# Zhiyu014/GNN-UDS

Hardware: AMD Instinct MI355X
Metric: graph-steps/sec (forward rollout), |V|=10k |E|=12k d=64 (higher is better)
Workload: dtype f32 storage/accumulate, GEMM operands as bf16 hi+lo split (3 MFMA products)

## Files before the change

### gnn_uds_amd/csrc/kernels_fused_ws.hpp

```cpp
#pragma once
#include "kernels_fused.hpp"

namespace uds {

#ifndef UDS_WS_NY
#define UDS_WS_NY 4
#endif
#ifndef UDS_WS_SLOTS
#define UDS_WS_SLOTS 4
#endif
constexpr int WS_NY = UDS_WS_NY, WS_NX = FUSED_WAVES - WS_NY;
#ifdef UDS_WS_YG
constexpr int WS_YG = UDS_WS_NY;
#else
constexpr int WS_YG = 0;
#endif
constexpr int WS_SLOTS = UDS_WS_SLOTS;
#ifndef UDS_WS_PRE
#define UDS_WS_PRE 0
#endif
constexpr int WS_PRE = UDS_WS_PRE;
static_assert(WS_PRE % WS_SLOTS == 0, "WS_PRE must be a multiple of WS_SLOTS");
#ifndef UDS_WS_XPRIO
#define UDS_WS_XPRIO 1
#endif
static_assert(WS_NY >= 2 && WS_NY <= 4, "2 .. 4 waves multiply the primary rows");

inline int64_t fused_ws_lds_bytes(int p_cap, int q_cap, int meta_cap) {
  return 4 * ((int64_t)meta_cap + 4 * p_cap + 3 * FUSED_D + FUSED_H + 2 * (int64_t)q_cap * SEC_STRIDE + 2 * (int64_t)p_cap * FUSED_D);
}

template <int IMM>
__device__ __forceinline__ void ws_gld16(f32x4 &dst, const float *base, unsigned voff) {
  asm volatile("global_load_dwordx4 %0, %1, %2 offset:%3" : "=v"(dst) : "v"(voff), "s"(base), "n"(IMM) : "memory");
}
__device__ __forceinline__ void ws_pin4(f32x4 &a0, f32x4 &a1, f32x4 &a2, f32x4 &a3) {
  asm volatile("" : "+v"(a0), "+v"(a1), "+v"(a2), "+v"(a3));
}
__device__ __forceinline__ void row8_max4(const float (&in)[4], float (&out)[4]) {
  asm("s_nop 1\n\t" UDS_DPP4_FIRST("v_max_f32_dpp", "quad_perm:[1,0,3,2]") UDS_DPP4("v_max_f32_dpp", "quad_perm:[2,3,0,1]")
      UDS_DPP4("v_max_f32_dpp", "row_half_mirror")
      : "=&v"(out[0]), "=&v"(out[1]), "=&v"(out[2]), "=&v"(out[3])
      : "v"(in[0]), "v"(in[1]), "v"(in[2]), "v"(in[3]));
}
__device__ __forceinline__ void row8_sum4(const float (&in)[4], float (&out)[4]) {
  asm("s_nop 1\n\t" UDS_DPP4_FIRST("v_add_f32_dpp", "quad_perm:[1,0,3,2]") UDS_DPP4("v_add_f32_dpp", "quad_perm:[2,3,0,1]")
      UDS_DPP4("v_add_f32_dpp", "row_half_mirror")
      : "=&v"(out[0]), "=&v"(out[1]), "=&v"(out[2]), "=&v"(out[3])
      : "v"(in[0]), "v"(in[1]), "v"(in[2]), "v"(in[3]));
}
template <int HI>
__device__ __forceinline__ unsigned ws_add_half(unsigned pk, unsigned base) {
  unsigned r;
  if (HI) asm("v_add_u32_sdwa %0, %1, %2 dst_sel:DWORD dst_unused:UNUSED_PAD src0_sel:WORD_1 src1_sel:DWORD" : "=v"(r) : "v"(pk), "v"(base));
  else asm("v_add_u32_sdwa %0, %1, %2 dst_sel:DWORD dst_unused:UNUSED_PAD src0_sel:WORD_0 src1_sel:DWORD" : "=v"(r) : "v"(pk), "v"(base));
  return r;
}
__device__ __forceinline__ void ws_vmcnt(int n) {
  switch (n) {
    case 0: asm volatile("s_waitcnt vmcnt(0)" ::: "memory"); break;
    case 1: asm volatile("s_waitcnt vmcnt(1)" ::: "memory"); break;
    case 2: asm volatile("s_waitcnt vmcnt(2)" ::: "memory"); break;
    case 3: asm volatile("s_waitcnt vmcnt(3)" ::: "memory"); break;
    case 4: asm volatile("s_waitcnt vmcnt(4)" ::: "memory"); break;
    case 5: asm volatile("s_waitcnt vmcnt(5)" ::: "memory"); break;
    case 6: asm volatile("s_waitcnt vmcnt(6)" ::: "memory"); break;
    case 7: asm volatile("s_waitcnt vmcnt(7)" ::: "memory"); break;
    default: asm volatile("s_waitcnt vmcnt(8)" ::: "memory"); break;
  }
}

template <int ACT>
__global__ __launch_bounds__(FUSED_WAVES * 64, 2) void k_fused_ws(FusedArgs a) {
  constexpr int NT = FUSED_WAVES * 64, NY = WS_NY, NX = WS_NX;
  constexpr int FP = 64, FS = 64;
  constexpr int KT_S = FS / 32, MB_S = FUSED_H / 16;
  constexpr int KT_X = FP / 32, KT_B = KT_X + 1, MB_B = FUSED_D / 16;
  constexpr int U = FUSED_U;
  constexpr int PJ = (8 + NY - 1) / NY;
  constexpr int SJ = (16 + NX - 1) / NX;
  extern __shared__ __attribute__((aligned(16))) int32_t smem[];

  const int tid = threadIdx.x, lane = tid & 63;
  const int wave = __builtin_amdgcn_readfirstlane(tid >> 6);
#ifdef UDS_WS_PAIR_SAME
  static_assert(NY == 4, "UDS_WS_PAIR_SAME assumes 4 + 4");
  const bool team_y = (wave & 3) < 2;
  const int yw = (wave & 1) + 2 * (wave >> 2), xw = ((wave & 3) - 2) + 2 * (wave >> 2);
#else
  const bool team_y = wave < NY;
  const int yw = wave, xw = wave - NY;
#endif
  const int r16 = lane & 15, qd = lane >> 4;
  const int c16 = r16, rs = qd;

  const int W = gridDim.x, b = blockIdx.x;
  const int q8 = W / 8, r8 = W % 8, xcd = b % 8;
  const int w = (xcd < r8 ? xcd * (q8 + 1) : r8 * (q8 + 1) + (xcd - r8) * q8) + b / 8;
  const int tile = w % a.n_tiles;
  const int chunk_id = w / a.n_tiles;
  const int s_begin = chunk_id * a.chunk;
  const int s_end = min(a.S, (chunk_id + 1) * a.chunk);
  const int sd = __builtin_amdgcn_readfirstlane(a.hdr[tile * TILE_HDR_INTS + 6]);
  if (!((a.side_mask >> sd) & 1)) return;
  const FusedSide &S_ = a.side[sd];

  float *s_self = reinterpret_cast<float *>(smem + a.meta_cap);
  float *s_nbr = s_self + 2 * a.p_cap;
  float *attn = s_nbr + 2 * a.p_cap;
  float *sec = attn + 3 * FUSED_D + FUSED_H;
  float *hx = sec + 2 * a.q_cap * SEC_STRIDE;
  const int sec_buf = a.q_cap * SEC_STRIDE, hx_buf = a.p_cap * FUSED_D;

  {
    const uint4 *src = reinterpret_cast<const uint4 *>(a.blocks + (int64_t)tile * a.meta_cap);
    uint4 *dst = reinterpret_cast<uint4 *>(smem);
    for (int i = tid; i < a.meta_cap / 4; i += NT) dst[i] = src[i];
  }
  if (tid < FUSED_D) {
    attn[tid] = S_.a_self[tid] * 1.44269504088896340736f;
    attn[FUSED_D + tid] = S_.a_nbr[tid] * 1.44269504088896340736f;
    if (tid < FUSED_H) attn[2 * FUSED_D + tid] = S_.b_small ? S_.b_small[tid] : 0.f;
    attn[2 * FUSED_D + FUSED_H + tid] = S_.b_out ? S_.b_out[tid] : 0.f;
  }
  __syncthreads();
  const int n_own = __builtin_amdgcn_readfirstlane(smem[0]), n_prim = __builtin_amdgcn_readfirstlane(smem[1]),
            n_sec = __builtin_amdgcn_readfirstlane(smem[2]), flags = __builtin_amdgcn_readfirstlane(smem[3]),
            n_ovf = __builtin_amdgcn_readfirstlane(smem[4]), n_adj = __builtin_amdgcn_readfirstlane(smem[5]),
            inc_width = __builtin_amdgcn_readfirstlane(smem[7]);
  const EllOffsets off = ell_offsets(n_own, n_prim, n_sec, flags, n_ovf, n_adj);
  const int32_t *prim_ids = smem + off.prim;
  const int32_t *sec_ids = smem + off.sec;
  const uint32_t *inc_loc = reinterpret_cast<const uint32_t *>(smem + off.inc_loc);
  int32_t *inc_w = smem + off.inc_w;
  const f32x4 *inc_val4 = reinterpret_cast<const f32x4 *>(inc_w);
  const unsigned char *adj_b = reinterpret_cast<const unsigned char *>(smem + off.adj);
  const int32_t *ovf_ptr = smem + off.ovf_ptr, *ovf_loc = smem + off.ovf_loc;
  int32_t *ovf_w = smem + off.ovf_w;
  const int32_t *adj_ptr = smem + off.adj_ptr, *adj_loc = smem + off.adj_loc;

  for (int i = tid; i < ELL_INC * n_prim; i += NT) {
    const int k = inc_w[i];
    reinterpret_cast<float *>(inc_w)[i] = k >= 0 ? S_.ne_val[k] : 0.f;
  }
  if (flags & ELL_FLAG_INC_OVF)
    for (int i = tid; i < n_ovf; i += NT) reinterpret_cast<float *>(ovf_w)[i] = S_.ne_val[ovf_w[i]];
  const float *ovf_val = reinterpret_cast<const float *>(ovf_w);

#ifdef UDS_PHASE_TIMING
  unsigned long long tm_[8] = {0, 0, 0, 0, 0, 0, 0, 0}, tl_ = clock64();
  const unsigned long long rt0_ = __builtin_amdgcn_s_memrealtime(), mt0_ = tl_;
#define WS_STAMP(k) do { const unsigned long long n_ = clock64(); tm_[k] += n_ - tl_; tl_ = n_; } while (0)
#define WS_DUMP() do { if (a.dbg && lane == 0) { unsigned long long *o = a.dbg + ((size_t)blockIdx.x * 8 + wave) * 16; \
    for (int q_ = 0; q_ < 7; ++q_) o[q_] = tm_[q_]; o[12] = wave; \
    o[15] = ((__builtin_amdgcn_s_memrealtime() - rt0_) << 32) | ((clock64() - mt0_) & 0xffffffffull); \
    o[7] = 1ull | ((unsigned long long)sd << 8) | ((unsigned long long)n_own << 16) | ((unsigned long long)n_prim << 32) | ((unsigned long long)n_sec << 48); } } while (0)
#else
#define WS_STAMP(k) do { } while (0)
#define WS_DUMP() do { } while (0)
#endif
  const int64_t sec_stride = (int64_t)S_.n_sec_glob * FS, prim_stride = (int64_t)S_.n_prim_glob * FP;
  const int n_snap = s_end - s_begin;

  __syncthreads();
  if (team_y) {
#ifndef UDS_WS_MFMA16
    typedef float f32x16 __attribute__((ext_vector_type(16)));
    constexpr int KT32 = (FP + FUSED_H) / 16, KX32 = FP / 16, MB32 = FUSED_D / 32;
    static_assert(NY == 4, "one 32-row block per Y wave: four waves cover p_cap = 128");
    const int n32 = lane & 31, hf = lane >> 5;
    bf16x8 wh[KT32][MB32], wl[KT32][MB32];
#pragma unroll
    for (int t = 0; t < KT32; ++t)
#pragma unroll
      for (int m = 0; m < MB32; ++m) {
        wh[t][m] = __builtin_bit_cast(bf16x8, S_.w_big32[((t * MB32 + m) * 2 + 0) * 64 + lane]);
        wl[t][m] = __builtin_bit_cast(bf16x8, S_.w_big32[((t * MB32 + m) * 2 + 1) * 64 + lane]);
      }
    const int lrow = 32 * yw + n32;
    const bool valid = lrow < n_prim;
    const int lr = min(lrow, n_prim - 1);
    const unsigned prow = (unsigned)prim_ids[lr] * FP + 8u * hf;
    f32x4 pp[2 * KX32];
    const bool has_rem = S_.rem != nullptr;
    const unsigned rrow = (unsigned)prim_ids[lr] * FUSED_H + 8u * hf;
    f32x4 rm[4] = {f32x4{0.f, 0.f, 0.f, 0.f}, f32x4{0.f, 0.f, 0.f, 0.f}, f32x4{0.f, 0.f, 0.f, 0.f}, f32x4{0.f, 0.f, 0.f, 0.f}};
    const int64_t rem_stride = (int64_t)S_.n_prim_glob * FUSED_H;
    const unsigned ag_locs = inc_loc[lr];
    const f32x4 ag_vals = inc_val4[lr];
    __builtin_amdgcn_s_waitcnt(0x0F70);
    if (n_snap > 0) {
      const float *base = S_.prim_in + s_begin * prim_stride;
      static_for<2 * KX32>([&](auto i_) {
        constexpr int i = decltype(i_)::value;
        pp[i] = *reinterpret_cast<const f32x4 *>(base + prow + 16 * (i >> 1) + 4 * (i & 1));
      });
      if (has_rem) {
        const float *rb = S_.rem + s_begin * rem_stride + rrow;
        rm[0] = *reinterpret_cast<const f32x4 *>(rb);
        rm[1] = *reinterpret_cast<const f32x4 *>(rb + 4);
        rm[2] = *reinterpret_cast<const f32x4 *>(rb + 16);
        rm[3] = *reinterpret_cast<const f32x4 *>(rb + 20);
      }
    }
    WS_STAMP(0);
    lds_barrier();

    auto mfma3_32 = [&](const bf16x8 &a_h, const bf16x8 &a_l, const bf16x8 &d_h, const bf16x8 &d_l, f32x16 acc) __attribute__((always_inline)) {
      acc = __builtin_amdgcn_mfma_f32_32x32x16_bf16(a_h, d_l, acc, 0, 0, 0);
      acc = __builtin_amdgcn_mfma_f32_32x32x16_bf16(a_l, d_h, acc, 0, 0, 0);
      acc = __builtin_amdgcn_mfma_f32_32x32x16_bf16(a_h, d_h, acc, 0, 0, 0);
      return acc;
    };
    for (int k = 0; k <= n_snap; ++k) {
#ifdef UDS_WS_ABL_NO_P2
      if (false) {
#else
      if (k < n_snap && 32 * yw < n_prim) {
#endif
        const bool more = k + 1 < n_snap;
        const float *next = S_.prim_in + (s_begin + k + 1) * prim_stride;
        const float *secr = sec + (k & 1) * sec_buf;
        float *hxw = hx + (k & 1) * hx_buf;
        float *ssw = s_self + (k & 1) * a.p_cap, *snw = s_nbr + (k & 1) * a.p_cap;
        bf16x8 dh[KT32], dl[KT32];
        static_for<KX32>([&](auto t_) {
          constexpr int t = decltype(t_)::value;
          const f32x4 u0 = pp[2 * t], u1 = pp[2 * t + 1];
          split8(make_float4(u0[0], u0[1], u0[2], u0[3]), make_float4(u1[0], u1[1], u1[2], u1[3]), dh[t], dl[t]);
        });
        if (more)
          static_for<2 * KX32>([&](auto i_) {
            constexpr int i = decltype(i_)::value;
            pp[i] = *reinterpret_cast<const f32x4 *>(next + prow + 16 * (i >> 1) + 4 * (i & 1));
          });
        f32x16 acc[MB32];
#pragma unroll
        for (int m = 0; m < MB32; ++m)
#pragma unroll
          for (int r = 0; r < 16; ++r) acc[m][r] = 0.f;
#pragma unroll
        for (int t = 0; t < KX32; ++t)
#pragma unroll
          for (int m = 0; m < MB32; ++m) acc[m] = mfma3_32(wh[t][m], wl[t][m], dh[t], dl[t], acc[m]);
        float4 g0 = make_float4(rm[0][0], rm[0][1], rm[0][2], rm[0][3]), g1 = make_float4(rm[1][0], rm[1][1], rm[1][2], rm[1][3]),
               g2 = make_float4(rm[2][0], rm[2][1], rm[2][2], rm[2][3]), g3 = make_float4(rm[3][0], rm[3][1], rm[3][2], rm[3][3]);
        if (more && has_rem) {
          const float *rb = S_.rem + (s_begin + k + 1) * rem_stride + rrow;
          rm[0] = *reinterpret_cast<const f32x4 *>(rb);
          rm[1] = *reinterpret_cast<const f32x4 *>(rb + 4);
          rm[2] = *reinterpret_cast<const f32x4 *>(rb + 16);
          rm[3] = *reinterpret_cast<const f32x4 *>(rb + 20);
        }
        auto fma4 = [&](float4 &g, float wv, const float4 &u) { g.x = fmaf(wv, u.x, g.x); g.y = fmaf(wv, u.y, g.y); g.z = fmaf(wv, u.z, g.z); g.w = fmaf(wv, u.w, g.w); };
        auto add_row = [&](unsigned la, float wa) {
          const float *ra = secr + la * SEC_STRIDE + 8 * hf;
          const float4 u0 = *reinterpret_cast<const float4 *>(ra), u1 = *reinterpret_cast<const float4 *>(ra + 4);
          const float4 u2 = *reinterpret_cast<const float4 *>(ra + 16), u3 = *reinterpret_cast<const float4 *>(ra + 20);
          fma4(g0, wa, u0); fma4(g1, wa, u1); fma4(g2, wa, u2); fma4(g3, wa, u3);
        };
        add_row(ag_locs & 0xffu, ag_vals[0]);
        add_row((ag_locs >> 8) & 0xffu, ag_vals[1]);
        if (inc_width > 2) {
          add_row((ag_locs >> 16) & 0xffu, ag_vals[2]);
          add_row(ag_locs >> 24, ag_vals[3]);
        }
        if (flags & ELL_FLAG_INC_OVF)
          for (int p = ovf_ptr[lr]; p < ovf_ptr[lr + 1]; ++p) add_row((unsigned)ovf_loc[p], ovf_val[p]);
        split8(g0, g1, dh[KX32], dl[KX32]);
        split8(g2, g3, dh[KX32 + 1], dl[KX32 + 1]);
#pragma unroll
        for (int t = KX32; t < KT32; ++t)
#pragma unroll
          for (int m = 0; m < MB32; ++m) acc[m] = mfma3_32(wh[t][m], wl[t][m], dh[t], dl[t], acc[m]);
        float ps = 0.f, pn = 0.f;
#pragma unroll
        for (int m = 0; m < MB32; ++m)
#pragma unroll
          for (int gq = 0; gq < 4; ++gq) {
            const f32x4 as4 = *reinterpret_cast<const f32x4 *>(attn + 32 * m + 8 * gq + 4 * hf);
            const f32x4 an4 = *reinterpret_cast<const f32x4 *>(attn + FUSED_D + 32 * m + 8 * gq + 4 * hf);
#pragma unroll
            for (int q = 0; q < 4; ++q) {
              ps = fmaf(acc[m][4 * gq + q], as4[q], ps);
              pn = fmaf(acc[m][4 * gq + q], an4[q], pn);
            }
          }
        ps += __shfl_xor(ps, 32);
        pn += __shfl_xor(pn, 32);
        if (valid) {
          if (hf == 0) {
            ssw[lrow] = ps;
            snw[lrow] = pn;
          }
#pragma unroll
          for (int m = 0; m < MB32; ++m)
#pragma unroll
            for (int gq = 0; gq < 4; ++gq) {
              const f32x4 o = {acc[m][4 * gq], acc[m][4 * gq + 1], acc[m][4 * gq + 2], acc[m][4 * gq + 3]};
              *reinterpret_cast<f32x4 *>(hxw + lrow * FUSED_D + (((8 * m + 2 * gq + hf) ^ (lrow & 7)) << 2)) = o;
            }
        }
      }
      WS_STAMP(1);
      lds_barrier();
      WS_STAMP(2);
    }
    WS_DUMP();
#else
    bf16x8 wbh[KT_B][MB_B], wbl[KT_B][MB_B];
#pragma unroll
    for (int t = 0; t < KT_B; ++t)
#pragma unroll
      for (int m = 0; m < MB_B; ++m) {
        wbh[t][m] = __builtin_bit_cast(bf16x8, S_.w_big[((t * MB_B + m) * 2 + 0) * 64 + lane]);
        wbl[t][m] = __builtin_bit_cast(bf16x8, S_.w_big[((t * MB_B + m) * 2 + 1) * 64 + lane]);
      }
    unsigned prow[PJ];
#pragma unroll
    for (int j = 0; j < PJ; ++j) prow[j] = (unsigned)prim_ids[min((yw + NY * j) * 16 + r16, n_prim - 1)] * FP + 4u * qd;
    f32x4 pp[PJ][2 * KT_X];
    unsigned ag_locs[PJ];
    f32x4 ag_vals[PJ];
#pragma unroll
    for (int j = 0; j < PJ; ++j) {
      const int lr = min((yw + NY * j) * 16 + r16, n_prim - 1);
      ag_locs[j] = inc_loc[lr];
      ag_vals[j] = inc_val4[lr];
    }
    const int yg_i = 4 * yw + rs, yg_ic = min(yg_i, n_own - 1);
    const bool yg_ok = WS_YG > 0 && yg_i < n_own;
    const unsigned yg_jb = adj_b[yg_ic * ELL_ADJ + c16];
    const bool yg_has = yg_ok && yg_jb != 0xFFu;
    const int yg_jn = yg_has ? (int)yg_jb : 0;
    const int yg_joff = yg_jn * (FUSED_D * 4) + ((yg_jn & 7) << 4);
    const int yg_orow = prim_ids[yg_ic] * FUSED_D + 4 * c16;
    int yg_dmax;
    {
      int dmx;
      if (flags & ELL_FLAG_LONG_ROWS) {
        dmx = yg_i < n_own ? adj_ptr[yg_ic + 1] - adj_ptr[yg_ic] : 0;
      } else {
        const unsigned long long m = __ballot(yg_i < n_own && adj_b[yg_ic * ELL_ADJ + c16] != 0xFF);
        dmx = __builtin_popcountll((m >> (16 * rs)) & 0xffffull);
      }
      dmx = max(dmx, __shfl_xor(dmx, 16));
      dmx = max(dmx, __shfl_xor(dmx, 32));
      yg_dmax = WS_YG > 0 ? __builtin_amdgcn_readfirstlane(dmx) : 0;
    }
    f32x4 bo = f32x4{0.f, 0.f, 0.f, 0.f};
    if (S_.b_out) bo = *reinterpret_cast<const f32x4 *>(S_.b_out + 4 * c16);
    auto phase3_y = [&](int s, int buf) __attribute__((always_inline)) {
      if (yg_dmax == 0) return;
      const float *hxr = hx + buf * hx_buf;
      const float *ssr = s_self + buf * a.p_cap, *snr = s_nbr + buf * a.p_cap;
      const float ss = ssr[yg_ic];
      f32x4 acc = f32x4{0.f, 0.f, 0.f, 0.f};
      float den;
      if (yg_dmax <= 16) {
        const float sv = ss + snr[yg_jn];
        const float lg = yg_has ? fmaxf(sv, 0.2f * sv) : -INFINITY;
        const float mx = row16_max(lg);
        const float ex = __builtin_amdgcn_exp2f(lg - mx);
        const float wgt = yg_has ? ex : 0.f;
        den = row16_sum(wgt);
        const char *hxb = reinterpret_cast<const char *>(hxr);
        const int cx = c16 << 4;
        int dmx = yg_dmax;
        asm volatile("" : "+s"(dmx));
        static_for<16 / WS_SLOTS>([&](auto t_) {
          constexpr int K = decltype(t_)::value * WS_SLOTS;
          if (K < dmx) {
            f32x4 hh[WS_SLOTS];
            static_for<WS_SLOTS>([&](auto i_) {
              constexpr int i = decltype(i_)::value;
              hh[i] = *reinterpret_cast<const f32x4 *>(hxb + (row16_bcast<K + i>(yg_joff) ^ cx));
            });
            static_for<WS_SLOTS>([&](auto i_) {
              constexpr int i = decltype(i_)::value;
              const float wv = __int_as_float(row16_bcast<K + i>(__float_as_int(wgt)));
#pragma unroll
              for (int q = 0; q < 4; ++q) acc[q] = fmaf(wv, hh[i][q], acc[q]);
            });
          }
        });
      } else {
        const int b0 = yg_ok ? adj_ptr[yg_i] : 0;
        const int dg = yg_ok ? adj_ptr[yg_i + 1] - b0 : 0;
        float mx = -INFINITY;
        for (int p = b0; p < b0 + dg; ++p) mx = fmaxf(mx, leaky02(ss + snr[adj_loc[p]]));
        den = 0.f;
        for (int p = b0; p < b0 + dg; ++p) {
          const int jj = adj_loc[p];
          const float wv = __builtin_amdgcn_exp2f(leaky02(ss + snr[jj]) - mx);
          const f32x4 hv = *reinterpret_cast<const f32x4 *>(hxr + jj * FUSED_D + ((c16 ^ (jj & 7)) << 2));
          den += wv;
#pragma unroll
          for (int q = 0; q < 4; ++q) acc[q] = fmaf(wv, hv[q], acc[q]);
        }
      }
      if (yg_ok) {
        const float inv = __builtin_amdgcn_rcpf(den);
        f32x4 o;
#pragma unroll
        for (int q = 0; q < 4; ++q) o[q] = fused_act<ACT>(fmaf(acc[q], inv, bo[q]), a.act);
        *reinterpret_cast<f32x4 *>(S_.out + ((int64_t)s * S_.n_prim_glob * FUSED_D + yg_orow)) = o;
      }
    };
    __builtin_amdgcn_s_waitcnt(0x0F70);
    if (n_snap > 0) {
      const float *base = S_.prim_in + s_begin * prim_stride;
      static_for<PJ>([&](auto j_) {
        constexpr int j = decltype(j_)::value;
        static_for<2 * KT_X>([&](auto c_) {
          constexpr int c = decltype(c_)::value;
          pp[j][c] = *reinterpret_cast<const f32x4 *>(base + prow[j] + 16 * c);
        });
      });
    }
    WS_STAMP(0);
    lds_barrier();

    for (int k = 0; k <= n_snap; ++k) {
#ifdef UDS_WS_ABL_NO_P2
      if (false) {
#else
      if (k < n_snap) {
#endif
        const bool more = k + 1 < n_snap;
        const float *next = S_.prim_in + (s_begin + k + 1) * prim_stride;
        const float *secr = sec + (k & 1) * sec_buf;
        float *hxw = hx + (k & 1) * hx_buf;
        float *ssw = s_self + (k & 1) * a.p_cap, *snw = s_nbr + (k & 1) * a.p_cap;
        static_for<PJ>([&](auto j_) {
          constexpr int j = decltype(j_)::value;
          const int blk = yw + NY * j;
#ifndef UDS_WS_P2_BRANCH
          {
#else
          if (blk * 16 < n_prim) {
#endif
            bf16x8 dh[KT_B], dl[KT_B];
            static_for<KT_X>([&](auto t_) {
              constexpr int t = decltype(t_)::value;
              const f32x4 u0 = pp[j][2 * t], u1 = pp[j][2 * t + 1];
              split8(make_float4(u0[0], u0[1], u0[2], u0[3]), make_float4(u1[0], u1[1], u1[2], u1[3]), dh[t], dl[t]);
            });
            if (more)
              static_for<2 * KT_X>([&](auto c_) {
                constexpr int c = decltype(c_)::value;
                pp[j][c] = *reinterpret_cast<const f32x4 *>(next + prow[j] + 16 * c);
              });
            const int lrow = blk * 16 + r16;
            const bool valid = lrow < n_prim;
            const int lr = min(lrow, n_prim - 1);
            f32x4 acc[MB_B];
#pragma unroll
            for (int m = 0; m < MB_B; ++m) acc[m] = f32x4{0.f, 0.f, 0.f, 0.f};
#ifndef UDS_WS_ABL_Y_NO_MFMA
#pragma unroll
            for (int t = 0; t < KT_X; ++t)
#pragma unroll
              for (int m = 0; m < MB_B; ++m) acc[m] = mfma3(wbh[t][m], wbl[t][m], dh[t], dl[t], acc[m]);
#else
#pragma unroll
            for (int m = 0; m < MB_B; ++m) acc[m] = f32x4{__builtin_bit_cast(float, (unsigned)dh[0][0] << 16), (float)m, __builtin_bit_cast(float, (unsigned)dl[1][0] << 16), 0.f};
#endif
            const unsigned locs = ag_locs[j];
            const f32x4 vals = ag_vals[j];
            float4 g0 = make_float4(0.f, 0.f, 0.f, 0.f), g1 = g0;
            auto fma_row = [&](float wv, const float4 &u0, const float4 &u1) {
              g0.x = fmaf(wv, u0.x, g0.x); g0.y = fmaf(wv, u0.y, g0.y); g0.z = fmaf(wv, u0.z, g0.z); g0.w = fmaf(wv, u0.w, g0.w);
              g1.x = fmaf(wv, u1.x, g1.x); g1.y = fmaf(wv, u1.y, g1.y); g1.z = fmaf(wv, u1.z, g1.z); g1.w = fmaf(wv, u1.w, g1.w);
            };
            auto add2 = [&](unsigned la, float wa, unsigned lb, float wb) {
              const float *ra = secr + la * SEC_STRIDE + 4 * qd, *rb = secr + lb * SEC_STRIDE + 4 * qd;
              const float4 a0 = *reinterpret_cast<const float4 *>(ra), a1 = *reinterpret_cast<const float4 *>(ra + 16);
              const float4 b0 = *reinterpret_cast<const float4 *>(rb), b1 = *reinterpret_cast<const float4 *>(rb + 16);
              fma_row(wa, a0, a1);
              fma_row(wb, b0, b1);
            };
#ifndef UDS_WS_ABL_Y_NO_AGG
            add2(locs & 0xffu, vals[0], (locs >> 8) & 0xffu, vals[1]);
            if (inc_width > 2) add2((locs >> 16) & 0xffu, vals[2], locs >> 24, vals[3]);
#else
            g0.x = vals[0]; g1.y = vals[1]; g0.z = __uint_as_float(locs);
#endif
            if (flags & ELL_FLAG_INC_OVF)
              for (int p = ovf_ptr[lr]; p < ovf_ptr[lr + 1]; ++p) {
                const float *ra = secr + ovf_loc[p] * SEC_STRIDE + 4 * qd;
                fma_row(ovf_val[p], *reinterpret_cast<const float4 *>(ra), *reinterpret_cast<const float4 *>(ra + 16));
              }
            split8(g0, g1, dh[KT_X], dl[KT_X]);
#ifndef UDS_WS_ABL_Y_NO_MFMA
#pragma unroll
            for (int m = 0; m < MB_B; ++m) acc[m] = mfma3(wbh[KT_X][m], wbl[KT_X][m], dh[KT_X], dl[KT_X], acc[m]);
#else
            acc[0][3] += __builtin_bit_cast(float, (unsigned)dh[KT_X][0] << 16) + __builtin_bit_cast(float, (unsigned)dl[KT_X][0] << 16);
#endif
            typedef float f32x2 __attribute__((ext_vector_type(2)));
            f32x2 ps2 = {0.f, 0.f}, pn2 = {0.f, 0.f};
#pragma unroll
            for (int m = 0; m < MB_B; ++m) {
              const f32x4 as4 = *reinterpret_cast<const f32x4 *>(attn + 16 * m + 4 * qd);
              const f32x4 an4 = *reinterpret_cast<const f32x4 *>(attn + FUSED_D + 16 * m + 4 * qd);
              ps2 = __builtin_elementwise_fma(acc[m].xy, as4.xy, ps2);
              pn2 = __builtin_elementwise_fma(acc[m].xy, an4.xy, pn2);
              ps2 = __builtin_elementwise_fma(acc[m].zw, as4.zw, ps2);
              pn2 = __builtin_elementwise_fma(acc[m].zw, an4.zw, pn2);
            }
            const float ps = quarters_sum(ps2.x + ps2.y);
            const float pn = quarters_sum(pn2.x + pn2.y);
#ifdef UDS_WS_ABL_Y_NO_HXW
            if (valid && ps == 12345.f) {
#else
            if (valid) {
#endif
              if (qd == 0) {
                ssw[lrow] = ps;
                snw[lrow] = pn;
              }
#pragma unroll
              for (int m = 0; m < MB_B; ++m)
                *reinterpret_cast<f32x4 *>(hxw + lrow * FUSED_D + (((4 * m + qd) ^ (lrow & 7)) << 2)) = acc[m];
            }
          }
        });
      }
      if (WS_YG > 0 && k >= 1) phase3_y(s_begin + k - 1, (k - 1) & 1);
      WS_STAMP(1);
      lds_barrier();
      WS_STAMP(2);
    }
    WS_DUMP();
#endif
  } else {
#ifndef UDS_WS_NO_PRIO
    __builtin_amdgcn_s_setprio(UDS_WS_XPRIO);
#endif
#ifndef UDS_WS_MFMA16
    typedef float f32x16 __attribute__((ext_vector_type(16)));
    constexpr int KS32 = FS / 16, SJ32 = (8 + NX - 1) / NX;
    const int n32 = lane & 31, hf = lane >> 5;
    bf16x8 w1h[KS32], w1l[KS32];
#pragma unroll
    for (int t = 0; t < KS32; ++t) {
      w1h[t] = __builtin_bit_cast(bf16x8, S_.w_small32[(t * 2 + 0) * 64 + lane]);
      w1l[t] = __builtin_bit_cast(bf16x8, S_.w_small32[(t * 2 + 1) * 64 + lane]);
    }
    unsigned srow[SJ32];
#pragma unroll
    for (int j = 0; j < SJ32; ++j) srow[j] = ((unsigned)sec_ids[min((xw + NX * j) * 32 + n32, n_sec - 1)] * FS + 8u * hf) * 4u;
    f32x4 sp[SJ32][2 * KS32];
    auto load_sec_at = [&](const float *base) __attribute__((always_inline)) {
      static_for<SJ32>([&](auto j_) {
        constexpr int j = decltype(j_)::value;
        ws_gld16<0>(sp[j][0], base, srow[j]);
        ws_gld16<16>(sp[j][1], base, srow[j]);
        ws_gld16<64>(sp[j][2], base, srow[j]);
        ws_gld16<80>(sp[j][3], base, srow[j]);
        ws_gld16<128>(sp[j][4], base, srow[j]);
        ws_gld16<144>(sp[j][5], base, srow[j]);
        ws_gld16<192>(sp[j][6], base, srow[j]);
        ws_gld16<208>(sp[j][7], base, srow[j]);
      });
    };
    auto load_sec = [&](int s) __attribute__((always_inline)) { load_sec_at(S_.sec_in + s * sec_stride); };
#define UDS_WS_RUNNING_PTRS 1
#else
    bf16x8 wsh[KT_S][MB_S], wsl[KT_S][MB_S];
#pragma unroll
    for (int t = 0; t < KT_S; ++t)
#pragma unroll
      for (int m = 0; m < MB_S; ++m) {
        wsh[t][m] = __builtin_bit_cast(bf16x8, S_.w_small[((t * MB_S + m) * 2 + 0) * 64 + lane]);
        wsl[t][m] = __builtin_bit_cast(bf16x8, S_.w_small[((t * MB_S + m) * 2 + 1) * 64 + lane]);
      }
    unsigned srow[SJ];
#pragma unroll
    for (int j = 0; j < SJ; ++j) srow[j] = ((unsigned)sec_ids[min((xw + NX * j) * 16 + r16, n_sec - 1)] * FS + 4u * qd) * 4u;
    f32x4 sp[SJ][2 * KT_S];
    auto load_sec = [&](int s) __attribute__((always_inline)) {
      const float *base = S_.sec_in + s * sec_stride;
      static_for<SJ>([&](auto j_) {
        constexpr int j = decltype(j_)::value;
        ws_gld16<0>(sp[j][0], base, srow[j]);
        ws_gld16<64>(sp[j][1], base, srow[j]);
        ws_gld16<128>(sp[j][2], base, srow[j]);
        ws_gld16<192>(sp[j][3], base, srow[j]);
      });
    };
#endif
#ifndef UDS_WS_OCT_WD
#define UDS_WS_OCT_WD 4
#endif
#ifndef UDS_WS_OCT_GRP
#define UDS_WS_OCT_GRP 1
#endif
#ifndef UDS_WS_P3_GROUPS
    const int ro = lane >> 3, c8 = lane & 7, hf8 = ro & 1;
    int p3_dmax[U];
    unsigned p3_pk[U][4];
    unsigned p3_jb4 = 0;
    int n_st = 0;
#pragma unroll
    for (int u = 0; u < U; ++u) {
      const int i = 8 * (NX * u + xw) + ro;
      const int ic = min(i, n_own - 1);
      int dmx;
      if (flags & ELL_FLAG_LONG_ROWS) {
        dmx = i < n_own ? adj_ptr[ic + 1] - adj_ptr[ic] : 0;
      } else {
        const unsigned long long m0 = __ballot(i < n_own && adj_b[ic * ELL_ADJ + c8] != 0xFF);
        const unsigned long long m1 = __ballot(i < n_own && adj_b[ic * ELL_ADJ + 8 + c8] != 0xFF);
        dmx = __builtin_popcountll((m0 >> (8 * ro)) & 0xffull) + __builtin_popcountll((m1 >> (8 * ro)) & 0xffull);
      }
#pragma unroll
      for (int o = 8; o < 64; o <<= 1) dmx = max(dmx, __shfl_xor(dmx, o));
      p3_dmax[u] = __builtin_amdgcn_readfirstlane(dmx);
#pragma unroll
      for (int k2 = 0; k2 < 4; ++k2) {
        unsigned pk = 0;
#pragma unroll
        for (int h = 0; h < 2; ++h) {
          const unsigned jb = adj_b[ic * ELL_ADJ + 2 * k2 + h];
          const unsigned j = (i < n_own && jb != 0xFFu) ? jb : 0u;
          pk |= (j * (FUSED_D * 4) + (((j & 7) ^ c8) << 4)) << (16 * h);
        }
        p3_pk[u][k2] = pk;
      }
      p3_jb4 |= (i < n_own ? (unsigned)adj_b[i * ELL_ADJ + c8] : 0xFFu) << (8 * u);
      if (8 * (NX * u + xw) < n_own) n_st += 2;
    }
    const float *bias_l = attn + 2 * FUSED_D + FUSED_H + 4 * c8;
    __builtin_amdgcn_s_waitcnt(0x0F70);
#else
    int p3_dmax[2][U];
    unsigned p3_jb[2][U];
    int p3_joff[2][U], p3_orow[2][U], p3_ic[2][U];
    int n_st = 0;
#pragma unroll
    for (int t = 0; t < 2; ++t)
#pragma unroll
      for (int u = 0; u < U; ++u) {
        const int i = 4 * (WS_YG + NX * (2 * u + t) + xw) + rs;
        const int ic = min(i, n_own - 1);
        int dmx;
        if (flags & ELL_FLAG_LONG_ROWS) {
          dmx = i < n_own ? adj_ptr[ic + 1] - adj_ptr[ic] : 0;
        } else {
          const unsigned long long m = __ballot(i < n_own && adj_b[ic * ELL_ADJ + c16] != 0xFF);
          dmx = __builtin_popcountll((m >> (16 * rs)) & 0xffffull);
        }
        dmx = max(dmx, __shfl_xor(dmx, 16));
        dmx = max(dmx, __shfl_xor(dmx, 32));
        p3_dmax[t][u] = __builtin_amdgcn_readfirstlane(dmx);
        p3_jb[t][u] = adj_b[ic * ELL_ADJ + c16];
        {
          const bool has_ = i < n_own && p3_jb[t][u] != 0xFFu;
          const int jn_ = has_ ? (int)p3_jb[t][u] : 0;
          p3_joff[t][u] = jn_ * (FUSED_D * 4) + ((jn_ & 7) << 4);
          p3_orow[t][u] = prim_ids[ic] * FUSED_D + 4 * c16;
          p3_ic[t][u] = ic;
        }
        if (4 * (WS_YG + NX * (2 * u + t) + xw) < n_own) ++n_st;
      }
    f32x4 bo = f32x4{0.f, 0.f, 0.f, 0.f};
    if (S_.b_out) bo = *reinterpret_cast<const f32x4 *>(S_.b_out + 4 * c16);
    __builtin_amdgcn_s_waitcnt(0x0F70);
#endif

#ifndef UDS_WS_MFMA16
    auto phase1 = [&](int buf) __attribute__((always_inline)) {
      float *secw = sec + buf * sec_buf;
      static_for<SJ32>([&](auto j_) {
        constexpr int j = decltype(j_)::value;
        const int blk = xw + NX * j;
        if (blk * 32 < n_sec) {
          f32x16 acc;
#pragma unroll
          for (int gq = 0; gq < 4; ++gq) {
            const f32x4 b4 = *reinterpret_cast<const f32x4 *>(attn + 2 * FUSED_D + 8 * gq + 4 * hf);
#pragma unroll
            for (int q = 0; q < 4; ++q) acc[4 * gq + q] = b4[q];
          }
          static_for<KS32>([&](auto t_) {
            constexpr int t = decltype(t_)::value;
            const f32x4 u0 = sp[j][2 * t], u1 = sp[j][2 * t + 1];
            bf16x8 dh, dl;
            split8(make_float4(u0[0], u0[1], u0[2], u0[3]), make_float4(u1[0], u1[1], u1[2], u1[3]), dh, dl);
            acc = __builtin_amdgcn_mfma_f32_32x32x16_bf16(w1h[t], dl, acc, 0, 0, 0);
            acc = __builtin_amdgcn_mfma_f32_32x32x16_bf16(w1l[t], dh, acc, 0, 0, 0);
            acc = __builtin_amdgcn_mfma_f32_32x32x16_bf16(w1h[t], dh, acc, 0, 0, 0);
          });
          const int lrow = blk * 32 + n32;
          if (lrow < n_sec) {
#pragma unroll
            for (int gq = 0; gq < 4; ++gq) {
              f32x4 o;
#pragma unroll
              for (int q = 0; q < 4; ++q) o[q] = fused_act<ACT>(acc[4 * gq + q], a.act);
              *reinterpret_cast<f32x4 *>(secw + lrow * SEC_STRIDE + 8 * gq + 4 * hf) = o;
            }
          }
        }
      });
    };
    auto pin_rows = [&]() __attribute__((always_inline)) {
      static_for<SJ32>([&](auto j_) {
        constexpr int j = decltype(j_)::value;
        ws_pin4(sp[j][0], sp[j][1], sp[j][2], sp[j][3]);
        ws_pin4(sp[j][4], sp[j][5], sp[j][6], sp[j][7]);
      });
    };
#else
    auto phase1 = [&](int buf) __attribute__((always_inline)) {
      float *secw = sec + buf * sec_buf;
      static_for<SJ>([&](auto j_) {
        constexpr int j = decltype(j_)::value;
        const int blk = xw + NX * j;
        if (blk * 16 < n_sec) {
          bf16x8 dh[KT_S], dl[KT_S];
          static_for<KT_S>([&](auto t_) {
            constexpr int t = decltype(t_)::value;
            const f32x4 u0 = sp[j][2 * t], u1 = sp[j][2 * t + 1];
            split8(make_float4(u0[0], u0[1], u0[2], u0[3]), make_float4(u1[0], u1[1], u1[2], u1[3]), dh[t], dl[t]);
          });
          const int lrow = blk * 16 + r16;
          f32x4 acc[MB_S];
#pragma unroll
          for (int m = 0; m < MB_S; ++m) acc[m] = *reinterpret_cast<const f32x4 *>(attn + 2 * FUSED_D + 16 * m + 4 * qd);
#pragma unroll
          for (int t = 0; t < KT_S; ++t)
#pragma unroll
            for (int m = 0; m < MB_S; ++m) acc[m] = mfma3(wsh[t][m], wsl[t][m], dh[t], dl[t], acc[m]);
          if (lrow < n_sec) {
#pragma unroll
            for (int m = 0; m < MB_S; ++m) {
              f32x4 o;
#pragma unroll
              for (int q = 0; q < 4; ++q) o[q] = fused_act<ACT>(acc[m][q], a.act);
              *reinterpret_cast<f32x4 *>(secw + lrow * SEC_STRIDE + 16 * m + 4 * qd) = o;
            }
          }
        }
      });
    };
    auto pin_rows = [&]() __attribute__((always_inline)) {
      static_for<SJ>([&](auto j_) {
        constexpr int j = decltype(j_)::value;
        ws_pin4(sp[j][0], sp[j][1], sp[j][2], sp[j][3]);
      });
    };

#endif

    if (n_snap > 0) {
      load_sec(s_begin);
      ws_vmcnt(0);
      pin_rows();
      phase1(0);
      if (n_snap > 1) load_sec(s_begin + 1);
    }
    WS_STAMP(0);
    lds_barrier();

#ifndef UDS_WS_P3_GROUPS
    auto phase3o = [&](float *out_snap, int buf) __attribute__((always_inline)) {
      const float *hxr = hx + buf * hx_buf;
      const float *ssr = s_self + buf * a.p_cap, *snr = s_nbr + buf * a.p_cap;
      int d0 = p3_dmax[0], d1 = p3_dmax[1], d2 = p3_dmax[2], d3 = p3_dmax[3];
      asm volatile("" : "+s"(d0), "+s"(d1), "+s"(d2), "+s"(d3));
      const int e3 = d3, e2 = max(e3, d2), e1 = max(e2, d1), e0 = max(e1, d0);
      if (e0 == 0) return;

      float ss[U], lg0[U], lg1[U], w0[U], w1[U], den[U];
      bool ok[U], has0[U], has1[U];
      unsigned jb0[U], jb1[U];
      int joff1[U];
#pragma unroll
      for (int u = 0; u < U; ++u) {
        ok[u] = 8 * (NX * u + xw) + ro < n_own;
        jb0[u] = (p3_jb4 >> (8 * u)) & 0xFFu;
        ss[u] = ssr[8 * (NX * u + xw) + ro];
      }
#pragma unroll
      for (int u = 0; u < U; ++u) has0[u] = ok[u] && jb0[u] != 0xFFu;
      f32x4 acc0[U], acc1[U];
#pragma unroll
      for (int u = 0; u < U; ++u) acc0[u] = acc1[u] = f32x4{0.f, 0.f, 0.f, 0.f};
      if (e0 <= 16) {
        const bool ext = e0 > 8;
        float sn[U];
#pragma unroll
        for (int u = 0; u < U; ++u) sn[u] = snr[jb0[u]];
        asm volatile("" : "+v"(sn[0]), "+v"(sn[1]), "+v"(sn[2]), "+v"(sn[3]));
#pragma unroll
        for (int u = 0; u < U; ++u) {
          const float sv = ss[u] + sn[u];
          lg0[u] = has0[u] ? fmaxf(sv, 0.2f * sv) : -INFINITY;
        }
        float mx[U];
        row8_max4(lg0, mx);
        if (ext) {
          float m1[U];
#pragma unroll
          for (int u = 0; u < U; ++u) jb1[u] = adj_b[(8 * (NX * u + xw) + ro) * ELL_ADJ + 8 + c8];
          asm volatile("" : "+v"(jb1[0]), "+v"(jb1[1]), "+v"(jb1[2]), "+v"(jb1[3]));
#pragma unroll
          for (int u = 0; u < U; ++u) sn[u] = snr[jb1[u]];
          asm volatile("" : "+v"(sn[0]), "+v"(sn[1]), "+v"(sn[2]), "+v"(sn[3]));
#pragma unroll
          for (int u = 0; u < U; ++u) {
            has1[u] = ok[u] && jb1[u] != 0xFFu;
            const int j1 = has1[u] ? (int)jb1[u] : 0;
            joff1[u] = j1 * (FUSED_D * 4) + ((j1 & 7) << 4);
            const float sv = ss[u] + sn[u];
            lg1[u] = has1[u] ? fmaxf(sv, 0.2f * sv) : -INFINITY;
          }
          row8_max4(lg1, m1);
#pragma unroll
          for (int u = 0; u < U; ++u) mx[u] = fmaxf(mx[u], m1[u]);
        }
#pragma unroll
        for (int u = 0; u < U; ++u) w0[u] = has0[u] ? __builtin_amdgcn_exp2f(lg0[u] - mx[u]) : 0.f;
        row8_sum4(w0, den);
        if (ext) {
          float d1s[U];
#pragma unroll
          for (int u = 0; u < U; ++u) w1[u] = has1[u] ? __builtin_amdgcn_exp2f(lg1[u] - mx[u]) : 0.f;
          row8_sum4(w1, d1s);
#pragma unroll
          for (int u = 0; u < U; ++u) den[u] += d1s[u];
        }
        typedef const __attribute__((address_space(3))) f32x4 *lds_f4;
        const unsigned hxa0 = lds_addr(hxr) + 128 * hf8, hxa1 = lds_addr(hxr) + 128 - 128 * hf8;
        const int cx = c8 << 4;
        const int bp = (lane & 56) << 2;
        using I1 = std::integral_constant<int, 1>; using I2 = std::integral_constant<int, 2>;
        using I3 = std::integral_constant<int, 3>; using I4 = std::integral_constant<int, 4>;
        auto step = [&](auto SET_, auto K_, auto A_) __attribute__((always_inline)) {
          constexpr int SET = decltype(SET_)::value, K = decltype(K_)::value, A = decltype(A_)::value,
                        Wd = (8 - K < UDS_WS_OCT_WD ? 8 - K : UDS_WS_OCT_WD);
          constexpr int G = UDS_WS_OCT_GRP;
          static_for<(A + G - 1) / G>([&](auto g_) {
            constexpr int u0 = decltype(g_)::value * G, GA = (A - u0 < G ? A - u0 : G);
            f32x4 h0[GA][Wd], h1[GA][Wd];
            static_for<GA>([&](auto u_) {
              constexpr int ul = decltype(u_)::value, u = u0 + ul;
              static_for<Wd>([&](auto i_) {
                constexpr int i = decltype(i_)::value, k = K + i;
                unsigned ad = 0;
                if (SET) ad = (unsigned)__builtin_amdgcn_ds_bpermute(bp + 4 * k, joff1[u]) ^ cx;
                unsigned ad0, ad1;
                if (SET) {
                  ad0 = ad + hxa0;
                  ad1 = ad + hxa1;
                } else {
                  ad0 = ws_add_half<k & 1>(p3_pk[u][k >> 1], hxa0);
                  ad1 = ws_add_half<k & 1>(p3_pk[u][k >> 1], hxa1);
                }
                h0[ul][i] = *(lds_f4)(uintptr_t)ad0;
                h1[ul][i] = *(lds_f4)(uintptr_t)ad1;
              });
            });
            static_for<GA>([&](auto u_) {
              constexpr int ul = decltype(u_)::value, u = u0 + ul;
              static_for<Wd>([&](auto i_) {
                constexpr int i = decltype(i_)::value, k = K + i;
                float wv;
                if (SET) wv = __int_as_float(__builtin_amdgcn_ds_bpermute(bp + 4 * k, __float_as_int(w1[u])));
                else {
                  const int wi = __float_as_int(w0[u]);
                  int t = __builtin_amdgcn_update_dpp(wi, wi, 0x150 + k, 0xf, 0xf, true);
                  t = __builtin_amdgcn_update_dpp(t, wi, 0x150 + 8 + k, 0xf, 0xc, false);
                  wv = __int_as_float(t);
                }
#pragma unroll
                for (int q = 0; q < 4; ++q) {
                  acc0[u][q] = fmaf(wv, h0[ul][i][q], acc0[u][q]);
                  acc1[u][q] = fmaf(wv, h1[ul][i][q], acc1[u][q]);
                }
              });
            });
          });
        };
        static_for<(8 + UDS_WS_OCT_WD - 1) / UDS_WS_OCT_WD>([&](auto t_) {
          constexpr int K = decltype(t_)::value * UDS_WS_OCT_WD;
          using IK = std::integral_constant<int, K>;
          using S0 = std::integral_constant<int, 0>;
          if (K < e3) step(S0{}, IK{}, I4{});
          else if (K < e2) step(S0{}, IK{}, I3{});
          else if (K < e1) step(S0{}, IK{}, I2{});
          else if (K < e0) step(S0{}, IK{}, I1{});
        });
        if (ext)
          static_for<(8 + UDS_WS_OCT_WD - 1) / UDS_WS_OCT_WD>([&](auto t_) {
            constexpr int K = decltype(t_)::value * UDS_WS_OCT_WD;
            using IK = std::integral_constant<int, K>;
            using S1 = std::integral_constant<int, 1>;
            if (K + 8 < e3) step(S1{}, IK{}, I4{});
            else if (K + 8 < e2) step(S1{}, IK{}, I3{});
            else if (K + 8 < e1) step(S1{}, IK{}, I2{});
            else if (K + 8 < e0) step(S1{}, IK{}, I1{});
          });
      } else {
#pragma unroll
        for (int u = 0; u < U; ++u) {
          const int i = 8 * (NX * u + xw) + ro;
          const int b0 = i < n_own ? adj_ptr[i] : 0;
          const int dg = i < n_own ? adj_ptr[i + 1] - b0 : 0;
          float mx = -INFINITY;
          for (int p = b0; p < b0 + dg; ++p) mx = fmaxf(mx, leaky02(ss[u] + snr[adj_loc[p]]));
          den[u] = 0.f;
          for (int p = b0; p < b0 + dg; ++p) {
            const int jj = adj_loc[p];
            const float wv = __builtin_amdgcn_exp2f(leaky02(ss[u] + snr[jj]) - mx);
            const f32x4 v0 = *reinterpret_cast<const f32x4 *>(hxr + jj * FUSED_D + 32 * hf8 + ((c8 ^ (jj & 7)) << 2));
            const f32x4 v1 = *reinterpret_cast<const f32x4 *>(hxr + jj * FUSED_D + 32 - 32 * hf8 + ((c8 ^ (jj & 7)) << 2));
            den[u] += wv;
#pragma unroll
            for (int q = 0; q < 4; ++q) {
              acc0[u][q] = fmaf(wv, v0[q], acc0[u][q]);
              acc1[u][q] = fmaf(wv, v1[q], acc1[u][q]);
            }
          }
        }
      }
      f32x4 bo0 = *reinterpret_cast<const f32x4 *>(bias_l + 32 * hf8), bo1 = *reinterpret_cast<const f32x4 *>(bias_l + 32 - 32 * hf8);
      int pid[U];
#pragma unroll
      for (int u = 0; u < U; ++u) pid[u] = prim_ids[8 * (NX * u + xw) + ro];
      asm volatile("" : "+v"(pid[0]), "+v"(pid[1]), "+v"(pid[2]), "+v"(pid[3]), "+v"(bo0), "+v"(bo1));
      float *out_s = out_snap + (4 * c8 + 32 * hf8);
      const int o1_off = 32 - 64 * hf8;
#pragma unroll
      for (int u = 0; u < U; ++u) {
        if (ok[u]) {
          const float inv = __builtin_amdgcn_rcpf(den[u]);
          f32x4 o0, o1;
#pragma unroll
          for (int q = 0; q < 4; ++q) {
            o0[q] = fused_act<ACT>(fmaf(acc0[u][q], inv, bo0[q]), a.act);
            o1[q] = fused_act<ACT>(fmaf(acc1[u][q], inv, bo1[q]), a.act);
          }
          float *orow = out_s + (int64_t)pid[u] * FUSED_D;
          *reinterpret_cast<f32x4 *>(orow) = o0;
          *reinterpret_cast<f32x4 *>(orow + o1_off) = o1;
        }
      }
    };
#else
    auto phase3 = [&](int TR, int s, int buf) __attribute__((always_inline)) {
#define P3S(arr, u) (TR ? arr[1][u] : arr[0][u])
      const float *hxr = hx + buf * hx_buf;
      const float *ssr = s_self + buf * a.p_cap, *snr = s_nbr + buf * a.p_cap;
      int jn[U], dmax[U], orow[U];
      float ss[U], lg[U], wgt[U], den[U];
      bool ok[U], has[U];
      int dm = 0;
#pragma unroll
      for (int u = 0; u < U; ++u) {
        const int i = 4 * (WS_YG + NX * (2 * u + TR) + xw) + rs;
        const int ic = min(i, n_own - 1);
        ok[u] = i < n_own;
        has[u] = ok[u] && P3S(p3_jb, u) != 0xFFu;
        jn[u] = has[u] ? (int)P3S(p3_jb, u) : 0;
        dmax[u] = P3S(p3_dmax, u);
        ss[u] = ssr[P3S(p3_ic, u)];
        orow[u] = P3S(p3_orow, u);
        dm = max(dm, dmax[u]);
      }
      if (dm == 0) return;
      f32x4 acc[U];
#pragma unroll
      for (int u = 0; u < U; ++u) acc[u] = f32x4{0.f, 0.f, 0.f, 0.f};
      if (dm <= 16) {
        int d0 = dmax[0], d1 = dmax[1], d2 = dmax[2], d3 = dmax[3];
        asm volatile("" : "+s"(d0), "+s"(d1), "+s"(d2), "+s"(d3));
        const int e3 = d3, e2 = max(e3, d2), e1 = max(e2, d1), e0 = max(e1, d0);
        const char *hxb = reinterpret_cast<const char *>(hxr);
        const int cx = c16 << 4;
        int joff[U];
#pragma unroll
        for (int u = 0; u < U; ++u) {
          joff[u] = P3S(p3_joff, u);
          const float sv = ss[u] + snr[jn[u]];
          const float sc = fmaxf(sv, 0.2f * sv);
          lg[u] = has[u] ? sc : -INFINITY;
        }
        using I1 = std::integral_constant<int, 1>; using I2 = std::integral_constant<int, 2>;
        using I3 = std::integral_constant<int, 3>; using I4 = std::integral_constant<int, 4>;
        constexpr int R = WS_PRE > 0 ? WS_PRE : 1;
        f32x4 hh0[U][R];
        auto pre_read = [&](auto K_, auto A_) __attribute__((always_inline)) {
          constexpr int K = decltype(K_)::value, A = decltype(A_)::value;
          static_for<A>([&](auto u_) {
            constexpr int u = decltype(u_)::value;
            hh0[u][K] = *reinterpret_cast<const f32x4 *>(hxb + (row16_bcast<K>(joff[u]) ^ cx));
          });
        };
        if constexpr (WS_PRE > 0)
          static_for<WS_PRE>([&](auto K_) {
            constexpr int K = decltype(K_)::value;
            if (K < e3) pre_read(K_, I4{});
            else if (K < e2) pre_read(K_, I3{});
            else if (K < e1) pre_read(K_, I2{});
            else if (K < e0) pre_read(K_, I1{});
          });
        static_assert(U == 4, "the four-at-once reductions below");
        float mx[U];
        row16_max4(lg, mx);
#pragma unroll
        for (int u = 0; u < U; ++u) {
          const float ex = __builtin_amdgcn_exp2f(lg[u] - mx[u]);
          wgt[u] = has[u] ? ex : 0.f;
        }
        row16_sum4(wgt, den);
        auto pre_fma = [&](auto K_, auto A_) __attribute__((always_inline)) {
          constexpr int K = decltype(K_)::value, A = decltype(A_)::value;
          static_for<A>([&](auto u_) {
            constexpr int u = decltype(u_)::value;
            const float wv = __int_as_float(row16_bcast<K>(__float_as_int(wgt[u])));
#pragma unroll
            for (int q = 0; q < 4; ++q) acc[u][q] = fmaf(wv, hh0[u][K][q], acc[u][q]);
          });
        };
        if constexpr (WS_PRE > 0)
          static_for<WS_PRE>([&](auto K_) {
            constexpr int K = decltype(K_)::value;
            if (K < e3) pre_fma(K_, I4{});
            else if (K < e2) pre_fma(K_, I3{});
            else if (K < e1) pre_fma(K_, I2{});
            else if (K < e0) pre_fma(K_, I1{});
          });
        auto step = [&](auto K_, auto A_) __attribute__((always_inline)) {
          constexpr int K = decltype(K_)::value, A = decltype(A_)::value, Wd = WS_SLOTS;
          f32x4 hh[A][Wd];
#pragma unroll
          for (int u = 0; u < A; ++u)
            static_for<Wd>([&](auto i_) {
              constexpr int i = decltype(i_)::value;
              hh[u][i] = *reinterpret_cast<const f32x4 *>(hxb + (row16_bcast<K + i>(joff[u]) ^ cx));
            });
#pragma unroll
          for (int u = 0; u < A; ++u)
            static_for<Wd>([&](auto i_) {
              constexpr int i = decltype(i_)::value;
              const float wv = __int_as_float(row16_bcast<K + i>(__float_as_int(wgt[u])));
#pragma unroll
              for (int q = 0; q < 4; ++q) acc[u][q] = fmaf(wv, hh[u][i][q], acc[u][q]);
            });
        };
        bool more = e0 > WS_PRE;
        static_for<(16 - WS_PRE) / WS_SLOTS>([&](auto t_) {
          constexpr int K = WS_PRE + decltype(t_)::value * WS_SLOTS;
          if (more) {
            using IK = std::integral_constant<int, K>;
#ifdef UDS_WS_P3_FLAT
            step(IK{}, I4{});
#else
            if (K < e3) step(IK{}, I4{});
// ... 93 lines not shown
```

Baseline: 299,700.

## Overlap kernel setup loads: prefetch tile metadata, defer ne_val gathers into Y waves

Restructures the kernel prologue so that the first uint4 of the tile metadata and the attention/bias parameters are loaded into registers before the side check and barrier. The block-wide pass that resolves incidence ids to ne_val weights in LDS is removed. Instead, each Y lane gathers its own four values after issuing its prim/rem loads, and the overflow entries are resolved by Y waves only. On the X side, the first secondary-feature load is issued before the small-weight loads and the adjacency setup, and the explicit vmcnt(0) wait is dropped. The aim is to hide global-load latency behind setup work and remove one __syncthreads. The cost is added dependence on waitcnt placement, and the code now relies on pin_rows to enforce completion of the secondary loads. Overflow values are written by Y waves only, with the X waves synchronized through the later lds_barrier.

```diff
diff --git a/gnn_uds_amd/csrc/kernels_fused_ws.hpp b/gnn_uds_amd/csrc/kernels_fused_ws.hpp
--- a/gnn_uds_amd/csrc/kernels_fused_ws.hpp
+++ b/gnn_uds_amd/csrc/kernels_fused_ws.hpp
@@ -101,6 +101,22 @@
   const int chunk_id = w / a.n_tiles;
   const int s_begin = chunk_id * a.chunk;
   const int s_end = min(a.S, (chunk_id + 1) * a.chunk);
+#ifdef UDS_PHASE_TIMING
+  unsigned long long tm_[8] = {0, 0, 0, 0, 0, 0, 0, 0}, tl_ = clock64();
+  const unsigned long long rt0_ = __builtin_amdgcn_s_memrealtime(), mt0_ = tl_;
+#define WS_STAMP(k) do { const unsigned long long n_ = clock64(); tm_[k] += n_ - tl_; tl_ = n_; } while (0)
+#define WS_DUMP() do { if (a.dbg && lane == 0) { unsigned long long *o = a.dbg + ((size_t)blockIdx.x * 8 + wave) * 16; \
+    for (int q_ = 0; q_ < 7; ++q_) o[q_] = tm_[q_]; o[12] = wave; \
+    o[15] = ((__builtin_amdgcn_s_memrealtime() - rt0_) << 32) | ((clock64() - mt0_) & 0xffffffffull); \
+    o[7] = 1ull | ((unsigned long long)sd << 8) | ((unsigned long long)n_own << 16) | ((unsigned long long)n_prim << 32) | ((unsigned long long)n_sec << 48); } } while (0)
+#else
+#define WS_STAMP(k) do { } while (0)
+#define WS_DUMP() do { } while (0)
+#endif
+  const int n4 = a.meta_cap / 4;
+  const uint4 *blk_src = reinterpret_cast<const uint4 *>(a.blocks + (int64_t)tile * a.meta_cap);
+  uint4 blk0 = make_uint4(0u, 0u, 0u, 0u);
+  if (tid < n4) blk0 = blk_src[tid];
   const int sd = __builtin_amdgcn_readfirstlane(a.hdr[tile * TILE_HDR_INTS + 6]);
   if (!((a.side_mask >> sd) & 1)) return;
   const FusedSide &S_ = a.side[sd];
@@ -111,17 +127,26 @@
   float *sec = attn + 3 * FUSED_D + FUSED_H;
   float *hx = sec + 2 * a.q_cap * SEC_STRIDE;
   const int sec_buf = a.q_cap * SEC_STRIDE, hx_buf = a.p_cap * FUSED_D;
-
+  const int64_t sec_stride = (int64_t)S_.n_sec_glob * FS, prim_stride = (int64_t)S_.n_prim_glob * FP;
+  const int n_snap = s_end - s_begin;
+
+  float at_s = 0.f, at_n = 0.f, at_bs = 0.f, at_bo = 0.f;
+  if (tid < FUSED_D) {
+    at_s = S_.a_self[tid];
+    at_n = S_.a_nbr[tid];
+    if (tid < FUSED_H && S_.b_small) at_bs = S_.b_small[tid];
+    if (S_.b_out) at_bo = S_.b_out[tid];
+  }
   {
-    const uint4 *src = reinterpret_cast<const uint4 *>(a.blocks + (int64_t)tile * a.meta_cap);
     uint4 *dst = reinterpret_cast<uint4 *>(smem);
-    for (int i = tid; i < a.meta_cap / 4; i += NT) dst[i] = src[i];
+    if (tid < n4) dst[tid] = blk0;
+    for (int i = tid + NT; i < n4; i += NT) dst[i] = blk_src[i];
   }
   if (tid < FUSED_D) {
-    attn[tid] = S_.a_self[tid] * 1.44269504088896340736f;
-    attn[FUSED_D + tid] = S_.a_nbr[tid] * 1.44269504088896340736f;
-    if (tid < FUSED_H) attn[2 * FUSED_D + tid] = S_.b_small ? S_.b_small[tid] : 0.f;
-    attn[2 * FUSED_D + FUSED_H + tid] = S_.b_out ? S_.b_out[tid] : 0.f;
+    attn[tid] = at_s * 1.44269504088896340736f;
+    attn[FUSED_D + tid] = at_n * 1.44269504088896340736f;
+    if (tid < FUSED_H) attn[2 * FUSED_D + tid] = at_bs;
+    attn[2 * FUSED_D + FUSED_H + tid] = at_bo;
   }
   __syncthreads();
   const int n_own = __builtin_amdgcn_readfirstlane(smem[0]), n_prim = __builtin_amdgcn_readfirstlane(smem[1]),
@@ -133,36 +158,23 @@
   const int32_t *sec_ids = smem + off.sec;
   const uint32_t *inc_loc = reinterpret_cast<const uint32_t *>(smem + off.inc_loc);
   int32_t *inc_w = smem + off.inc_w;
-  const f32x4 *inc_val4 = reinterpret_cast<const f32x4 *>(inc_w);
   const unsigned char *adj_b = reinterpret_cast<const unsigned char *>(smem + off.adj);
   const int32_t *ovf_ptr = smem + off.ovf_ptr, *ovf_loc = smem + off.ovf_loc;
   int32_t *ovf_w = smem + off.ovf_w;
+  const float *ovf_val = reinterpret_cast<const float *>(ovf_w);
   const int32_t *adj_ptr = smem + off.adj_ptr, *adj_loc = smem + off.adj_loc;
-
+#if !defined(UDS_WS_MFMA16) && !defined(UDS_WS_P3_GROUPS)
+#define UDS_WS_FAST_SETUP 1
+#else
+  const f32x4 *inc_val4 = reinterpret_cast<const f32x4 *>(inc_w);
   for (int i = tid; i < ELL_INC * n_prim; i += NT) {
     const int k = inc_w[i];
     reinterpret_cast<float *>(inc_w)[i] = k >= 0 ? S_.ne_val[k] : 0.f;
   }
   if (flags & ELL_FLAG_INC_OVF)
     for (int i = tid; i < n_ovf; i += NT) reinterpret_cast<float *>(ovf_w)[i] = S_.ne_val[ovf_w[i]];
-  const float *ovf_val = reinterpret_cast<const float *>(ovf_w);
-
-#ifdef UDS_PHASE_TIMING
-  unsigned long long tm_[8] = {0, 0, 0, 0, 0, 0, 0, 0}, tl_ = clock64();
-  const unsigned long long rt0_ = __builtin_amdgcn_s_memrealtime(), mt0_ = tl_;
-#define WS_STAMP(k) do { const unsigned long long n_ = clock64(); tm_[k] += n_ - tl_; tl_ = n_; } while (0)
-#define WS_DUMP() do { if (a.dbg && lane == 0) { unsigned long long *o = a.dbg + ((size_t)blockIdx.x * 8 + wave) * 16; \
-    for (int q_ = 0; q_ < 7; ++q_) o[q_] = tm_[q_]; o[12] = wave; \
-    o[15] = ((__builtin_amdgcn_s_memrealtime() - rt0_) << 32) | ((clock64() - mt0_) & 0xffffffffull); \
-    o[7] = 1ull | ((unsigned long long)sd << 8) | ((unsigned long long)n_own << 16) | ((unsigned long long)n_prim << 32) | ((unsigned long long)n_sec << 48); } } while (0)
-#else
-#define WS_STAMP(k) do { } while (0)
-#define WS_DUMP() do { } while (0)
-#endif
-  const int64_t sec_stride = (int64_t)S_.n_sec_glob * FS, prim_stride = (int64_t)S_.n_prim_glob * FP;
-  const int n_snap = s_end - s_begin;
-
   __syncthreads();
+#endif
   if (team_y) {
 #ifndef UDS_WS_MFMA16
     typedef float f32x16 __attribute__((ext_vector_type(16)));
@@ -187,8 +199,12 @@
     f32x4 rm[4] = {f32x4{0.f, 0.f, 0.f, 0.f}, f32x4{0.f, 0.f, 0.f, 0.f}, f32x4{0.f, 0.f, 0.f, 0.f}, f32x4{0.f, 0.f, 0.f, 0.f}};
     const int64_t rem_stride = (int64_t)S_.n_prim_glob * FUSED_H;
     const unsigned ag_locs = inc_loc[lr];
+#ifdef UDS_WS_FAST_SETUP
+    const int4 ag_ids = reinterpret_cast<const int4 *>(inc_w)[lr];
+#else
     const f32x4 ag_vals = inc_val4[lr];
     __builtin_amdgcn_s_waitcnt(0x0F70);
+#endif
     if (n_snap > 0) {
       const float *base = S_.prim_in + s_begin * prim_stride;
       static_for<2 * KX32>([&](auto i_) {
@@ -203,6 +219,17 @@
         rm[3] = *reinterpret_cast<const f32x4 *>(rb + 20);
       }
     }
+#ifdef UDS_WS_FAST_SETUP
+    f32x4 ag_vals;
+    ag_vals[0] = ag_ids.x >= 0 ? S_.ne_val[ag_ids.x] : 0.f;
+    ag_vals[1] = ag_ids.y >= 0 ? S_.ne_val[ag_ids.y] : 0.f;
+    ag_vals[2] = ag_ids.z >= 0 ? S_.ne_val[ag_ids.z] : 0.f;
+    ag_vals[3] = ag_ids.w >= 0 ? S_.ne_val[ag_ids.w] : 0.f;
+    if (flags & ELL_FLAG_INC_OVF)
+#pragma nounroll
+      for (int i = 64 * yw + lane; i < n_ovf; i += 64 * NY) reinterpret_cast<float *>(ovf_w)[i] = S_.ne_val[ovf_w[i]];
+    __builtin_amdgcn_s_waitcnt(0x0F70);
+#endif
     WS_STAMP(0);
     lds_barrier();
 
@@ -542,12 +569,14 @@
     typedef float f32x16 __attribute__((ext_vector_type(16)));
     constexpr int KS32 = FS / 16, SJ32 = (8 + NX - 1) / NX;
     const int n32 = lane & 31, hf = lane >> 5;
+#ifndef UDS_WS_FAST_SETUP
     bf16x8 w1h[KS32], w1l[KS32];
 #pragma unroll
     for (int t = 0; t < KS32; ++t) {
       w1h[t] = __builtin_bit_cast(bf16x8, S_.w_small32[(t * 2 + 0) * 64 + lane]);
       w1l[t] = __builtin_bit_cast(bf16x8, S_.w_small32[(t * 2 + 1) * 64 + lane]);
     }
+#endif
     unsigned srow[SJ32];
 #pragma unroll
     for (int j = 0; j < SJ32; ++j) srow[j] = ((unsigned)sec_ids[min((xw + NX * j) * 32 + n32, n_sec - 1)] * FS + 8u * hf) * 4u;
@@ -599,6 +628,15 @@
 #endif
 #ifndef UDS_WS_P3_GROUPS
     const int ro = lane >> 3, c8 = lane & 7, hf8 = ro & 1;
+#ifdef UDS_WS_FAST_SETUP
+    if (n_snap > 0) load_sec(s_begin);
+    bf16x8 w1h[KS32], w1l[KS32];
+#pragma unroll
+    for (int t = 0; t < KS32; ++t) {
+      w1h[t] = __builtin_bit_cast(bf16x8, S_.w_small32[(t * 2 + 0) * 64 + lane]);
+      w1l[t] = __builtin_bit_cast(bf16x8, S_.w_small32[(t * 2 + 1) * 64 + lane]);
+    }
+#endif
     int p3_dmax[U];
     unsigned p3_pk[U][4];
     unsigned p3_jb4 = 0;
@@ -756,8 +794,10 @@
 #endif
 
     if (n_snap > 0) {
+#ifndef UDS_WS_FAST_SETUP
       load_sec(s_begin);
       ws_vmcnt(0);
+#endif
       pin_rows();
       phase1(0);
       if (n_snap > 1) load_sec(s_begin + 1);
```

New measurement: 293,400. -2.1%, worse.
